# MinghanLi/STMask

Hardware: AMD Instinct MI355X
Metric: frames/sec at 360x640 R50-DCN-FPN (STMask hot path, fp32) (higher is better)
Workload: dtype f32

## Files before the change

include/stmask_hip.h:

```cpp
#ifndef STMASK_HIP_H_
#define STMASK_HIP_H_

#include <stddef.h>
#include <stdint.h>

#ifdef __cplusplus
extern "C" {
#endif

#define STM_ABI_VERSION 6

enum stm_status {
    STM_OK = 0,
    STM_EINVAL = -1,
    STM_ENULL = -2,
    STM_ELAUNCH = -3,
    STM_EWORKSPACE = -4,
    STM_EUNSUPPORTED = -5
};

typedef void* stm_stream_t;

int stm_version(void);
const char* stm_last_error_string(void);
// ... 150 lines not shown
int stm_conv_kxr_tile_pixels(int kw, int fmt, int channel_tiles);
size_t stm_conv_kxr_packed_bytes(const struct stm_conv_geom* g);
int stm_conv_pack_weights_kxr_f32(const float* weight, void* packed, const struct stm_conv_geom* g, float wscale, stm_stream_t stream);
int stm_conv2d_planar_kxr_f32(const void* x_planes, const void* packed_weight, const float* bias, float* out_f32, void* out_planes,
                              const struct stm_conv_geom* g, int relu, stm_stream_t stream);

size_t stm_chain_tail_weight_bytes(void);
size_t stm_chain_tail_weight_bytes_proj(void);
int stm_chain_pack_tail_f32(const float* w3, const float* w1_next, void* packed, float wscale3, float wscale1, stm_stream_t stream);
int stm_chain_pack_tail_proj_f32(const float* w3, const float* wds, const float* w1_next, void* packed, float wscale3, float wscale1,
                                 stm_stream_t stream);
int stm_bottleneck_chain_f32(const void* mid1_planes, const void* x_planes, void* y_planes, void* z_planes, const void* w2_packed,
                             const void* tail_packed, const float* b2, const float* b3, const float* b1_next, float out_scale2,
                             float out_scale3, float out_scale1, int B, int H, int W, stm_stream_t stream);
int stm_bottleneck_chain_proj_f32(const void* mid1_planes, const void* x0_planes, void* y_planes, void* z_planes, const void* w2_packed,
                                  const void* tail_packed, const float* b2, const float* b3, const float* b1_next, float out_scale2,
                                  float out_scale3, float out_scale1, int B, int H, int W, stm_stream_t stream);

size_t stm_conv_packed_weight_bytes(int Cout, int Cin, int kh, int kw, int planes);
int stm_conv_pack_weights_f32(const float* weight, void* packed, int Cout, int Cin, int kh, int kw, int planes,
                              stm_stream_t stream);
size_t stm_conv_packed_weight_bytes_tiled(int Cout, int Cin, int kh, int kw, int planes, int tile_n);
int stm_conv_pack_weights_tiled_f32(const float* weight, void* packed, int Cout, int Cin, int kh, int kw, int planes,
                                    int tile_n, stm_stream_t stream);
int stm_conv_pack_weights_fmt_f32(const float* weight, void* packed, int Cout, int Cin, int kh, int kw, int tile_n, int fmt,
                                  float wscale, stm_stream_t stream);
int stm_split_planes_fmt_f32(const float* x, void* planes, int64_t n_pixels, int C, int fmt, stm_stream_t stream);

int stm_split_bf16_planes_f32(const float* x , void* planes ,
                              int64_t n_pixels, int C, stm_stream_t stream);
int stm_conv2d_planar_f32(const void* x_planes, const void* packed_weight, const float* bias, const float* residual_f32,
                          const void* residual_planes, float* out_f32, void* out_planes, const stm_conv_geom* g, int relu,
                          stm_stream_t stream);
int stm_conv2d_planar_ws_f32(const void* x_planes, const void* packed_weight, const float* bias, const float* residual_f32,
                             const void* residual_planes, float* out_f32, void* out_planes, const stm_conv_geom* g, int relu,
                             void* workspace, size_t workspace_bytes, stm_stream_t stream);

int stm_gather_detections_f32(const int64_t* idx, const int64_t* cls, const float* score, const float* box, const int* count,
                              const float* mask_coeff, const float* track, const float* centerness, int B, int top_k, int N,
                              int mask_dim, int embed_dim, int D, float* out_box, int64_t* out_cls, float* out_score,
                              float* out_coeff, float* out_track, float* out_centerness, int* out_clip, stm_stream_t stream);
int stm_shift_rois_f32(const float* box, const int* clip, float* rois, int n, int feat_h, int feat_w, stm_stream_t stream);
int stm_shift_apply_f32(const float* loc_shift, const float* coeff_shift, float* box, float* coeff, float* score, int n,
                        int mask_dim, float score_decay, stm_stream_t stream);
int stm_match_scores_f32(const float* cos, const float* mask_iou, const float* det_box, const float* prev_box,
                         const float* det_score, const int64_t* det_cls, const int64_t* prev_cls, const int* det_clip,
                         const int* prev_offsets, int D, int Pn, const float* coeff4, float dummy_iou, int* match,
                         stm_stream_t stream);
int stm_match_scores_embed_f32(const float* det_track, const float* prev_track, int embed_dim, const float* mask_iou,
                               const float* det_box, const float* prev_box, const float* det_score, const int64_t* det_cls,
                               const int64_t* prev_cls, const int* det_clip, const int* prev_offsets, int D, int Pn,
                               const float* coeff4, float dummy_iou, int* match, stm_stream_t stream);
int stm_gather_rows2(const void* const* a_rows, const void* const* b_rows, void* const* out_rows, const int* row_bytes,
                     int n_tensors, const int* plan, int n_rows, int n_a, stm_stream_t stream);
int stm_pack_tracked_f32(const float* mask, const float* score, const int* tracked, const int* offsets, const float* box,
                         const int64_t* cls, const float* mask_coeff, int n_rows, int hw, int B, int top_k, int cols,
                         int mask_dim, int max_age, float score_thr, int* keep_ws, float* out, stm_stream_t stream);
int stm_pack_tracked_bits_f32(const uint64_t* mask_bits, int words, const float* score, const int* tracked, const int* offsets,
                              const float* box, const int64_t* cls, const float* mask_coeff, int n_rows, int B, int top_k,
                              int cols, int mask_dim, int max_age, float score_thr, int* keep_ws, float* out,
                              stm_stream_t stream);

int stm_split_planes_f16(const float* x, void* planes, int64_t n_pixels, int C, stm_stream_t stream);
int stm_conv_pack_weights_f16(const float* weight, void* packed, int Cout, int Cin, int kh, int kw, int tile_n, float wscale,
                              stm_stream_t stream);
int stm_conv2d_planar_f16(const void* x_planes, const void* packed_weight, const float* bias, const float* residual_f32,
// ... 169 lines not shown
```

stmask_amd/csrc/conv_bf16x.hip:

```cpp
#include "planar_common.h"
#include "conv_plan.h"
#include <stdarg.h>
#include <algorithm>
#include <array>
#include <type_traits>
#include <utility>
#include <atomic>

namespace {

static int* g_range_flags[STM_MAX_DEVICES] = {};
static int* current_range_flag()
{
    const int dev = stm_current_device();
    return dev >= 0 ? g_range_flags[dev] : nullptr;
}

struct PlanarArgs {
    const uint8_t* xp;
    const uint8_t* wp;
    const float* bias;
    const float* res_f32;
    const uint8_t* res_pl;
    float* out_f32;
// ... 190 lines not shown
    f16x8 r0[LPR], r1[LPR];
    if (pre) {
#pragma unroll
        for (int pass = 0; pass < LPR; ++pass) {
            const int m = min(m0 + wm * 64 + pass * (64 / LPR) + prow, a.M - 1);
            const size_t ri = (((size_t)(co >> 5) * a.res_np + m) * 32 + (co & 31)) * 2;
            r0[pass] = *reinterpret_cast<const f16x8*>(a.res_pl + ri);
            r1[pass] = fmt == 1 ? *reinterpret_cast<const f16x8*>(a.res_pl + ri + a.res_pstride) : r0[pass];
        }
    }
#pragma unroll
    for (int pass = 0; pass < LPR; ++pass) {
        const int pr = pass * (64 / LPR) + prow;
        const int m = m0 + wm * 64 + pr;
        if (m >= a.M) continue;
        const f32x4 v0 = *reinterpret_cast<const f32x4*>(park + pr * EP_LD + seg * 8);
        const f32x4 v1 = *reinterpret_cast<const f32x4*>(park + pr * EP_LD + seg * 8 + 4);
        float v[8] = {v0.x, v0.y, v0.z, v0.w, v1.x, v1.y, v1.z, v1.w};
#pragma unroll
        for (int e = 0; e < 8; ++e) v[e] = __builtin_fmaf(v[e], a.out_scale, bias8[e]);
        if (pre) epilogue_store8<false, FMT>(a, m, co, nvalid, v, true, r0[pass], r1[pass]);
        else epilogue_store8<false, FMT>(a, m, co, nvalid, v);
    }
}

__global__ __launch_bounds__(256) void planar_splitk_finish_kernel(const PlanarArgs a, int bn)
{
    const int segs_g = (a.cout_g + 7) >> 3;
    const int64_t idx = (int64_t)blockIdx.x * 256 + threadIdx.x;
    const int64_t total = (int64_t)a.M * a.groups * segs_g;
    if (idx >= total) return;
    const int sg = (int)(idx % (a.groups * segs_g));
    const int m = (int)(idx / (a.groups * segs_g));
    const int grp = sg / segs_g, cog = (sg - grp * segs_g) * 8;
    const int col = grp * a.ntpg * bn + cog;
    float v[8] = {0, 0, 0, 0, 0, 0, 0, 0};
    const float* p = a.partial + (size_t)m * a.ldp + col;
    const size_t pstride = (size_t)a.M * a.ldp;
    for (int k0 = 0; k0 < a.splitk; k0 += 4) {
        f32x4 q0[4], q1[4];
#pragma unroll
        for (int j = 0; j < 4; ++j) {
            const float* pk = p + (size_t)min(k0 + j, a.splitk - 1) * pstride;
            q0[j] = *reinterpret_cast<const f32x4*>(pk);
            q1[j] = *reinterpret_cast<const f32x4*>(pk + 4);
        }
#pragma unroll
        for (int j = 0; j < 4; ++j) {
            if (k0 + j < a.splitk) {
                v[0] += q0[j].x; v[1] += q0[j].y; v[2] += q0[j].z; v[3] += q0[j].w;
                v[4] += q1[j].x; v[5] += q1[j].y; v[6] += q1[j].z; v[7] += q1[j].w;
            }
        }
    }
    epilogue_store8(a, m, grp * a.cout_g + cog, min(8, a.cout_g - cog), v);
}

constexpr int POOL_BIG_SHIFT = 16;
constexpr float POOL_BIG_PIECE = (float)(1 << POOL_BIG_SHIFT);
template <bool BIG>
__device__ __forceinline__ bool pooled_walk(const PlanarArgs& a, unsigned long long* pool, int pool_ld, const float* park, int lane, int mw, int col)
{
    constexpr int EP_LD = 32 * 2 + 4;
    const int hw = a.Ho * a.Wo;
    const int rows = min(64, a.M - mw);
    int b = mw / hw, r = mw - b * hw;
// ... 17 lines not shown
                while (!__hip_atomic_compare_exchange_weak(word, &old, old + add, __ATOMIC_RELAXED, __ATOMIC_RELAXED, __HIP_MEMORY_SCOPE_AGENT)) {}
                const unsigned long long now = old + add, margin = (unsigned long long)a.win_hw << (32 + POOL_BIG_SHIFT);
                if ((now < old || now >= 0ull - margin) && a.range_flag) *reinterpret_cast<volatile int*>(a.range_flag) = 1;
            }
            sum = 0.0f;
            if (r == hw) { r = 0; ++b; }
        }
    }
    return any_big;
}
__device__ __forceinline__ void pooled_epilogue(const PlanarArgs& a, unsigned long long* pool, int pool_ld, uint8_t* smem, int wave, int lane, int mw, int col)
{
    const float* park = park_base<2>(smem, wave);
    asm volatile("s_waitcnt lgkmcnt(0)" ::: "memory");
    if (pooled_walk<false>(a, pool, pool_ld, park, lane, mw, col)) pooled_walk<true>(a, pool, pool_ld, park, lane, mw, col);
}

template <int NPL, int MG, int NJ, int DT = 0, int ST = 2, int ABL = 0, bool DUAL = false, int CLS = 0>
__global__ __launch_bounds__(512, 1) void conv_planar_kernel(const typename planar_args<CLS>::type a_in)
{
#if defined(__HIP_DEVICE_COMPILE__)
    extern __shared__ __align__(16) uint8_t smem[];
    constexpr int BM = CV_BM * MG;
    constexpr int BN = 64 * NJ;
    constexpr int WPL = BN * 64;
    constexpr int XBUF = NPL * BM * 64, WBUF = NPL * WPL, BUF = XBUF + WBUF;
    constexpr int NWAVES = 4 * MG;
    constexpr int WDMA = (BN / 16) * NPL / NWAVES;
    static_assert((BN / 16) * NPL % NWAVES == 0, "weight tile must split evenly over the waves");
    static_assert(ST == 2 || (ST == 3 && DT == 1 && NPL <= 2), "the three-buffer ring is built for the fp16 formats");

    int tiles_ = a_in.m_tiles * a_in.n_tiles * a_in.splitk;
    if constexpr (CLS) tiles_ = a_in.cls_tiles;
    else if (a_in.m_gate) tiles_ = min(a_in.m_tiles, (*a_in.m_gate + BM - 1) / BM) * a_in.n_tiles;
    const int tiles = tiles_;
    const int per_xcd = (tiles + 7) >> 3;
    if (!CLS && a_in.m_gate && (int)(blockIdx.x >> 3) >= per_xcd) return;
    int logical = (blockIdx.x & 7) * per_xcd + (blockIdx.x >> 3);
    if constexpr (CLS) {
        const int j = blockIdx.x >> 3;
        const int jm = j / a_in.n_tiles, nt_ = j - jm * a_in.n_tiles;
        logical = (jm * 8 + (int)(blockIdx.x & 7)) * a_in.n_tiles + nt_;
    }
    if (logical >= tiles) return;
    PlanarArgs a_cls;
    const PlanarArgs* ap = &a_in;
    if constexpr (CLS) {
        int c = 0;
#pragma unroll
        for (int i = 1; i < 9; ++i)
            if (i < a_in.n_cls && logical >= a_in.cls[i].tile0) c = i;
        a_cls = static_cast<const PlanarArgs&>(a_in);
        a_cls.wp = a_in.cls[c].wp;
        a_cls.kh = a_in.cls[c].kh; a_cls.kw = a_in.cls[c].kw; a_cls.ph = a_in.cls[c].ph; a_cls.pw = a_in.cls[c].pw;
        a_cls.Ho = a_in.cls[c].Ho; a_cls.Wo = a_in.cls[c].Wo; a_cls.M = a_in.cls[c].M;
        a_cls.slabs = a_in.cls[c].slabs; a_cls.kslabs = a_in.cls[c].slabs; a_cls.win_off = a_in.cls[c].win_off;
        a_cls.inv_hw = a_in.cls[c].inv_hw; a_cls.inv_w = a_in.cls[c].inv_w;
        if constexpr (CLS == 2) {
            a_cls.xp = a_in.xp + a_in.x_off[c];
            a_cls.plane_bytes = a_in.plane_bytes - (unsigned)a_in.x_off[c];
            a_cls.m_gate = a_in.gate[c];
        }
        logical -= a_in.cls[c].tile0;
        ap = &a_cls;
    }
    const PlanarArgs& a = *ap;
    const int ksp = a.splitk == 1 ? 0 : logical % a.splitk;
// ... 906 lines not shown
    }
    const int out_ld = g->out_ld ? g->out_ld : g->Cout, res_ld = g->res_ld ? g->res_ld : g->Cout;
    STM_REQUIRE(out_ld >= g->Cout && res_ld >= g->Cout, STM_EINVAL, "%s: bad leading dimensions out_ld=%d res_ld=%d", who, out_ld, res_ld);
    const bool win = g->n_levels <= 0 && g->win_w > 0;
    const int64_t out_rows = win ? (int64_t)g->B * g->win_h * g->win_w : M;
    const int64_t x_np = g->x_np ? g->x_np : in_pixels, out_np = g->out_np ? g->out_np : out_rows, res_np = g->res_np ? g->res_np : M;
    STM_REQUIRE(!win || (!c.residual_f32 && !c.residual_planes && !dual), STM_EUNSUPPORTED, "%s: window launches take no residual / second source", who);
    STM_REQUIRE(x_np >= in_pixels && out_np >= out_rows && res_np >= M, STM_EINVAL, "%s: x_np / out_np / res_np smaller than the pixel count", who);
    STM_REQUIRE((uintptr_t)c.x_planes % 16 == 0 && (uintptr_t)c.packed_weight % 16 == 0, STM_EINVAL,
                "%s: x_planes and packed_weight must be 16-byte aligned", who);
    if (dual) {
        STM_REQUIRE(groups == 1 && g->n_levels <= 0 && g->kh == 1 && g->kw == 1 && g->sh == 1 && g->sw == 1 && g->ph == 0 && g->pw == 0 &&
                    g->H == g->Ho && g->W == g->Wo && (g->fmt == 1 || g->fmt == 2), STM_EUNSUPPORTED,
                    "%s: 1x1 / stride 1 / one group / fp16 plane formats only", who);
        STM_REQUIRE(dual->C2 > 0 && dual->C2 % CV_BK == 0 && dual->C2 < g->C && dual->s2 >= 1 && dual->H2 > 0 && dual->W2 > 0 &&
                    (dual->H2 - 1) / dual->s2 + 1 == g->Ho && (dual->W2 - 1) / dual->s2 + 1 == g->Wo, STM_EINVAL,
                    "%s: second source %d channels of %dx%d at stride %d does not match the %dx%d output", who, dual->C2, dual->H2, dual->W2, dual->s2,
                    g->Ho, g->Wo);
    }
    const int64_t x_slabs = dual ? (int64_t)(g->C - dual->C2) / CV_BK : (int64_t)groups * (g->C / CV_BK);
    const int64_t plane_bytes = x_slabs * x_np * 64;
    STM_REQUIRE(plane_bytes < ((int64_t)1 << 31), STM_EUNSUPPORTED, "%s: plane larger than 2 GiB", who);
    STM_REQUIRE(M < ((int64_t)1 << 30), STM_EUNSUPPORTED, "%s: too many output pixels", who);
    const int64_t o_slabs = stm_cdiv(g->Cout, 32);
    const int64_t xps = g->x_plane_stride ? g->x_plane_stride : x_slabs * x_np * 32;
    const int64_t ops = g->out_plane_stride ? g->out_plane_stride : o_slabs * out_np * 32;
    const int64_t rps = g->res_plane_stride ? g->res_plane_stride : o_slabs * res_np * 32;
    STM_REQUIRE(xps % 8 == 0, STM_EINVAL, "%s: x_plane_stride must be a multiple of 8 elements", who);
    a.xp = static_cast<const uint8_t*>(c.x_planes); a.wp = static_cast<const uint8_t*>(c.packed_weight); a.bias = c.bias;
    a.res_f32 = c.residual_f32; a.res_pl = static_cast<const uint8_t*>(c.residual_planes);
    a.out_f32 = c.out_f32; a.out_pl = static_cast<uint8_t*>(c.out_planes);
    a.B = g->B; a.H = g->H; a.W = g->W; a.C = g->C; a.Ho = g->Ho; a.Wo = g->Wo; a.Cout = g->Cout;
    a.kh = g->kh; a.kw = g->kw; a.sh = g->sh; a.sw = g->sw; a.ph = g->ph; a.pw = g->pw;
    a.out_ld = out_ld; a.res_ld = res_ld; a.relu = c.relu;
    a.x_np = (int)x_np; a.out_np = (int)out_np; a.res_np = (int)res_np;
    a.M = (int)M; a.n_tiles = stm_cdiv(g->Cout, bn); a.m_tiles = 0; a.slabs = g->kh * g->kw * (g->C / CV_BK);
    a.plane_bytes = (unsigned)plane_bytes;
    a.x_pstride = xps * 2; a.out_pstride = ops * 2; a.res_pstride = rps * 2;
    a.groups = groups; a.cout_g = cout_g; a.ntpg = stm_cdiv(cout_g, bn);
    for (int i = 0; i < 8; ++i) a.group_real[i] = (i < groups && g->group_cout[i] > 0 && g->group_cout[i] < cout_g) ? g->group_cout[i] : cout_g;
    a.n_levels = g->n_levels > 0 ? g->n_levels : 0;
    for (int l = 0; l < 8; ++l) { a.lvl_start[l] = g->lvl_start[l]; a.lvl_h[l] = g->lvl_h[l]; a.lvl_w[l] = g->lvl_w[l]; }
    a.lvl_start[8] = g->lvl_start[8];
    a.vec_epilogue = (cout_g % 8 == 0) && (!c.out_f32 || out_ld % 4 == 0) && (!c.residual_f32 || res_ld % 4 == 0) && ((uintptr_t)c.out_f32 % 16 == 0) &&
                     ((uintptr_t)c.out_planes % 16 == 0) && ((uintptr_t)c.residual_f32 % 16 == 0) && ((uintptr_t)c.residual_planes % 16 == 0) &&
                     (ops % 8 == 0) && (rps % 8 == 0);
    STM_REQUIRE(g->kh * g->kw <= 32, STM_EUNSUPPORTED, "%s: more than 32 taps", who);
    a.pointwise = (g->n_levels <= 0 && !win && g->kh == 1 && g->kw == 1 && g->sh == 1 && g->sw == 1 && g->ph == 0 && g->pw == 0) ? 1 : 0;
    a.win_w = win ? g->win_w : 0; a.win_hw = win ? g->win_h * g->win_w : 0; a.win_off = win ? g->win_y0 * g->win_w + g->win_x0 : 0;
    a.inv_hw = g->n_levels > 0 ? 0.0f : 1.0f / (float)((int64_t)g->Ho * g->Wo);
    a.inv_w = g->n_levels > 0 ? 0.0f : 1.0f / (float)g->Wo;
    STM_REQUIRE(g->n_levels > 0 || M < ((int64_t)1 << 24), STM_EUNSUPPORTED, "%s: more than 2^24 output pixels in one launch", who);
    a.fmt = (g->fmt >= 0 && g->fmt <= 2) ? g->fmt : 0;
    a.out_fmt = g->out_fmt_plus1 > 0 ? g->out_fmt_plus1 - 1 : a.fmt;
    STM_REQUIRE(a.out_fmt >= 0 && a.out_fmt <= 2 && (a.out_fmt == a.fmt || (a.fmt == 2 && a.out_fmt == 1)), STM_EINVAL,
                "%s: output format %d cannot be produced by a format-%d layer", who, a.out_fmt, a.fmt);
    a.out_scale = (a.fmt >= 1 && g->out_scale > 0.0f) ? g->out_scale : 1.0f;
    a.range_flag = current_range_flag();
    const int want_planes = a.fmt == 0 ? 3 : (a.fmt == 1 ? 2 : 1);
    STM_REQUIRE(g->planes == want_planes || (a.fmt == 0 && g->planes == 2), STM_EINVAL, "%s: format %d has %d planes (planes = %d)", who, a.fmt,
                want_planes, g->planes);
    a.splitk = 1; a.kslabs = a.slabs; a.partial = nullptr; a.ldp = a.n_tiles * bn;
    a.m_gate = gate;
    STM_REQUIRE(!gate || !wset || !wset->pool, STM_EUNSUPPORTED, "%s: pooled window sets take no pixel gate", who);
    a.xp2 = nullptr; a.x2_pstride = 0; a.plane2_bytes = 0; a.c1_slabs = a.slabs; a.x2_np = 0; a.H2 = a.W2 = 0; a.s2 = 1;
    if (dual) {
        const int64_t in2 = (int64_t)g->B * dual->H2 * dual->W2;
        const int64_t np2 = dual->x2_np ? dual->x2_np : in2;
        const int64_t slabs2 = dual->C2 / CV_BK;
        const int64_t ps2 = dual->x2_plane_stride ? dual->x2_plane_stride : slabs2 * np2 * 32;
        STM_REQUIRE(np2 >= in2 && slabs2 * np2 * 64 < ((int64_t)1 << 31) && ps2 % 8 == 0 && (uintptr_t)dual->x2 % 16 == 0, STM_EINVAL,
                    "%s: bad second-source plane geometry", who);
        a.xp2 = static_cast<const uint8_t*>(dual->x2); a.x2_pstride = ps2 * 2; a.plane2_bytes = (unsigned)(slabs2 * np2 * 64);
        a.c1_slabs = (int)x_slabs; a.x2_np = (int)np2; a.H2 = dual->H2; a.W2 = dual->W2; a.s2 = dual->s2;
    }
    bool full = cout_g % 64 == 0;
    for (int gi = 0; gi < groups && gi < 8; ++gi) full = full && a.group_real[gi] == cout_g;
    f = ConvFacts{bn, a.fmt, g->planes, groups, cout_g, full, a.slabs, a.kh, a.kw, a.sh, a.sw, a.ph, a.pw, M, a.n_tiles, dual != nullptr, win, gate != nullptr,
                  c.workspace && (uintptr_t)c.workspace % 16 == 0, c.workspace_bytes, a.ldp};
    return STM_OK;
}

bool window_inside(const stm_conv_window& w, const stm_conv_geom* g)
{
    return w.Ho > 0 && w.Wo > 0 && w.y0 >= 0 && w.x0 >= 0 && w.y0 + w.Ho <= g->win_h && w.x0 + w.Wo <= g->win_w;
}
bool window_taps_inside(const stm_conv_window& w, const stm_conv_geom* g) { return conv_plan::taps_inside(w.kh, w.kw, w.ph, w.pw, w.Ho, w.Wo, g->H, g->W); }

int64_t fill_cls(PlanarArgsCls::Cls& c, const void* packed, const stm_conv_window& w, const stm_conv_geom* g, int images, int row0, int tile0)
{
    const int64_t Mc = (int64_t)images * w.Ho * w.Wo;
    c.wp = static_cast<const uint8_t*>(packed);
    c.kh = w.kh; c.kw = w.kw; c.ph = w.ph; c.pw = w.pw; c.Ho = w.Ho; c.Wo = w.Wo; c.M = (int)Mc;
    c.slabs = w.kh * w.kw * (g->C / CV_BK);
    c.win_off = row0 + w.y0 * g->win_w + w.x0;
    c.inv_hw = 1.0f / (float)(w.Ho * w.Wo); c.inv_w = 1.0f / (float)w.Wo;
    c.tile0 = tile0;
    return Mc;
}

int build_gated_set(const ConvCall& c, const char* who, const ConvFacts& f, const int* gate, Launch& l)
{
    const stm_conv_geom* const g = c.g;
    const WinSet* const wset = c.wset;
    PlanarArgsSeg& as = l.args;
    STM_REQUIRE(f.bn == 128 && as.fmt == 1 && !c.dual && f.win, STM_EUNSUPPORTED, "%s: window sets run on the 256 x 128 ring tiles of the fp16x2 format", who);
    STM_REQUIRE(g->B % wset->n == 0, STM_EINVAL, "%s: %d images are not %d equal segments", who, g->B, wset->n);
    const int seg_b = g->B / wset->n;
    as.m_gate = nullptr;
    as.pool = nullptr; as.pool_ld = 0;
    int t0 = 0;
    for (int i = 0; i < 9; ++i) {
// ... 34 lines not shown
        STM_REQUIRE((int64_t)g->B * w.Ho * w.Wo < ((int64_t)1 << 24), STM_EUNSUPPORTED, "%s: more than 2^24 output pixels in one window", who);
        const int k = conv_plan::window_takes_kx3(tn, w.kh, w.kw, w.ph, w.pw, w.Ho, w.Wo, g->H, g->W) ? 1 : 0;
        const int64_t Mc = fill_cls(L[k].args.cls[ncls[k]++], wset->packed[i], w, g, g->B, 0, t0[k]);
        t0[k] += stm_cdiv(Mc, 2 * CV_BM) * f.n_tiles;
    }
    for (int k = 0; k < 2; ++k) {
        if (!ncls[k]) continue;
        PlanarArgsCls& ac = L[k].args;
        for (int i = ncls[k]; i < 9; ++i) ac.cls[i] = ac.cls[0];
        ac.pool = wset->pool;
        ac.pool_ld = g->Cout;
        ac.n_cls = ncls[k];
        ac.cls_tiles = t0[k];
        L[k].plan = conv_plan::plan_window_set(k == 1, 1, k == 0 ? CLS_ABL : 0, t0[k], f.n_tiles, ac.kslabs);
        L[k].planned = true;
    }
    return STM_OK;
}

int conv2d_planar_impl(const ConvCall& c, stm_stream_t stream)
{
    const char* who = c.dual ? "stm_conv2d_planar_dual_f32" : "stm_conv2d_planar_f32";
    const int* const gate = stm_internal_take_pixel_gate();
    Launch L[2];
    PlanarArgs& a = L[0].args;
    ConvFacts f;
    int rc = planar_validate(c, who, gate, a, f);
    if (rc != STM_OK) return rc;
    if (c.wset) {
        rc = gate ? build_gated_set(c, who, f, gate, L[0]) : build_window_set(c, who, f, tunables(), L);
        if (rc != STM_OK) return rc;
    } else {
        const ConvPlan& p = L[0].plan = conv_plan::plan_conv(f, tunables());
        a.m_tiles = p.m_tiles; a.splitk = p.splitk; a.kslabs = p.kslabs;
        if (p.splitk > 1) a.partial = static_cast<float*>(c.workspace);
        L[0].planned = true;
    }
    for (const Launch& l : L) {
        if (!l.planned) continue;
        rc = run_launch(l, stream);
        if (rc != STM_OK) return rc;
    }
    if (a.splitk < 2) return STM_OK;
    const int64_t total = (int64_t)a.M * a.groups * ((a.cout_g + 7) / 8);
    if (t_plan_text) { t_plan_text->add("planar_splitk_finish_kernel grid=%d block=256 lds=0\n", stm_cdiv(total, 256)); return STM_OK; }
    hipLaunchKernelGGL(planar_splitk_finish_kernel, dim3(stm_cdiv(total, 256)), dim3(256), 0, stm_hs(stream), a, f.bn);
    STM_CHECK_LAUNCH("planar_splitk_finish_kernel");
    return STM_OK;
}

stm_conv_geom window0_geom(const stm_conv_geom* g, const stm_conv_window& w)
{
    stm_conv_geom g0 = *g;
    g0.kh = w.kh; g0.kw = w.kw; g0.ph = w.ph; g0.pw = w.pw;
    g0.Ho = w.Ho; g0.Wo = w.Wo; g0.win_y0 = w.y0; g0.win_x0 = w.x0;
    return g0;
}
}

extern "C" int stm_conv2d_planar_ws_f32(const void* x_planes, const void* packed_weight, const float* bias, const float* residual_f32,
                                        const void* residual_planes, float* out_f32, void* out_planes, const stm_conv_geom* g,
                                        int relu, void* workspace, size_t workspace_bytes, stm_stream_t stream)
{
    return conv2d_planar_impl({x_planes, packed_weight, bias, residual_f32, residual_planes, out_f32, out_planes, g, relu, workspace, workspace_bytes,
                               nullptr, nullptr}, stream);
}
// ... 93 lines not shown
```

stmask_amd/csrc/conv_plan.h:

```cpp
#pragma once
#include <algorithm>
#include <cstddef>
#include <cstdint>

namespace conv_plan {

constexpr int CV_RING64_SMALL = 512;
constexpr int CV_SK_TARGET = 256;
struct ConvTunables {
    int ring = 3;
    int ring64 = 3;
    int splitk = 0;
    int mg = 0;
    int abl = 0;
    int kx3 = 1;
};

constexpr int BM = 128;
constexpr int KX3_WBUF = 2 * 128 * 64;
constexpr int KX3_LDS_LOOP = 2 * 2 * 272 * 64 + 3 * KX3_WBUF;

inline int cdiv(int64_t a, int64_t b) { return (int)((a + b - 1) / b); }

struct ConvFacts {
    int bn;
    int fmt, planes;
    int groups, cout_g;
    bool full;
    int slabs;
    int kh, kw, sh, sw, ph, pw;
    int64_t M;
    int n_tiles;
    bool dual, win, gated;
    bool ws_usable;
    size_t ws_bytes;
    int ldp;
};

struct ConvPlan {
    bool kx3 = false;
    int npl = 0, mg = 0, nj = 0, dt = 0, st = 0, abl = 0;
    bool dual = false;
    int cls = 0;
    int m_tiles = 0, splitk = 1, kslabs = 0;
    unsigned grid = 0, block = 0;
    size_t lds = 0;
};

inline size_t planar_lds(int npl, int mg, int nj, int st)
{
    size_t lds = (size_t)st * (npl * BM * mg * 64 + npl * (64 * nj) * 64);
    const size_t park = (size_t)4 * mg * 64 * (32 * nj + 4) * sizeof(float);
    return lds < park ? park : lds;
}
inline size_t kx3_lds(bool win)
{
    if (win) return 2 * 2 * 384 * 64 + 3 * KX3_WBUF;
    return std::max<size_t>(8 * 64 * (64 + 4) * sizeof(float), (size_t)KX3_LDS_LOOP);
}

inline void plan_splitk(ConvPlan& p, const ConvFacts& f, const ConvTunables& tn, int tiles)
{
    if (f.gated) return;
    int sk = tn.splitk;
    if (sk <= 0) {
        sk = 1;
        if (f.bn == 64) {
            if (!f.full) {
                if (tiles <= 256 && f.slabs >= 24) sk = (int)std::min<int64_t>(std::min<int64_t>(8, 768 / tiles), f.slabs / 10);
            } else if (tiles <= 128 && f.slabs >= 24)
                sk = (int)std::min<int64_t>(std::min<int64_t>(8, CV_SK_TARGET / tiles), f.slabs / (tiles <= 40 ? 10 : 16));
        } else if (tiles < 128 && f.slabs >= 24) sk = (int)std::min<int64_t>(std::min<int64_t>(8, 256 / tiles), f.slabs / 12);
    }
    if (sk < 2) return;
    const int per = cdiv(f.slabs, sk);
    sk = cdiv(f.slabs, per);
    if (sk < 2 || !f.ws_usable || (size_t)sk * f.M * f.ldp * sizeof(float) > f.ws_bytes) return;
    p.splitk = sk; p.kslabs = per;
}

inline ConvPlan plan_conv(const ConvFacts& f, const ConvTunables& tn)
{
    ConvPlan p;
    p.npl = f.fmt == 2 ? 1 : (f.fmt == 1 ? 2 : (f.planes == 3 ? 3 : 2));
    p.dt = f.fmt >= 1 ? 1 : 0;
    p.dual = f.dual;
    p.kslabs = f.slabs;
    if (f.bn == 64) {
        p.mg = 1; p.nj = 1;
        p.m_tiles = cdiv(f.M, BM);
        plan_splitk(p, f, tn, p.m_tiles * f.n_tiles);
        const int tiles = p.m_tiles * f.n_tiles * p.splitk;
        const bool small_grid = tiles <= CV_RING64_SMALL;
        const bool ring = f.full && (tn.ring64 == 3 ? (small_grid || (p.splitk == 1 && f.slabs >= 12 && f.slabs <= 40)) : tn.ring64 == 4);
        p.st = (f.fmt >= 1 && ring) ? 3 : 2;
        p.grid = 8 * cdiv(tiles, 8);
    } else {
        const int64_t t2 = (int64_t)cdiv(f.M, 2 * BM) * f.n_tiles;
        p.mg = tn.mg ? tn.mg : (t2 >= 192 ? 2 : 1);
        p.nj = 2;
        p.m_tiles = cdiv(f.M, BM * p.mg);
        plan_splitk(p, f, tn, p.m_tiles * f.n_tiles);
        const int tiles = p.m_tiles * f.n_tiles * p.splitk;
        const bool ring = tn.ring == 3;
        p.grid = 8 * cdiv(tiles, 8);
#ifdef STM_ABLATE
        if (f.fmt == 1 && ring && p.mg == 2 && tn.abl) {
            const int abl = tn.abl;
            p.abl = (abl == 1 || abl == 2 || abl == 3 || abl == 5 || abl == 8 || abl == 16 || abl == 32 || abl == 64) ? abl : 7;
            p.st = 3; p.dual = false;
// ... 39 lines not shown
```

stmask_amd/planar.py:

```python
import ctypes
import functools
import os
from typing import Any, NamedTuple, Optional

import torch
import torch.nn.functional as F

from . import _lib, ops
from ._lib import StmError, call
from .ops import _pair


FMT = 0
BACKBONE_FMT = None

TILE64_MAX_SLABS = 8
FCB_PLANAR = True
STEM_PLANAR = True
C3DS_FUSED = True
STEM_FUSED = True
CONV_KXR = True
TN_BORDER = True
TN_POOL = True
CONV_CHAIN = True
# ... 148 lines not shown
        if out_planes is not None:
            g.out_np, g.out_plane_stride = out_planes.shape[2], out_planes.shape[1] * out_planes.shape[2] * 32
            if out_slab_off < 0 or out_slab_off + -(-self.O // 32) > out_planes.shape[1]:
                raise StmError(f"PlanarConv: {self.O} output channels from slab {out_slab_off} run past the {out_planes.shape[1]} slabs of out_planes")
            p_pl = out_planes.data_ptr() + (out_slab_off * g.out_np + out_off_p) * 64
        if out_f32 is not None:
            g.out_ld = out_f32.shape[-1]
            p_f32 = out_f32.data_ptr() + (out_off_f * g.out_ld + out_ch_off) * 4
        r32 = rpl = 0
        if residual is not None:
            if residual.dtype == dt:
                if residual.shape[0] < NP:
                    raise StmError(f"PlanarConv: residual has {residual.shape[0]} plane(s), format {self.fmt} reads {NP}")
                g.res_np, g.res_plane_stride = residual.shape[2], residual.shape[1] * residual.shape[2] * 32
                rpl = residual.data_ptr()
            else:
                g.res_ld = residual.shape[-1]
                r32 = residual.data_ptr()
        started = _timing_start()
        x_ptr = xp.data_ptr() + ((x_ch_off // 32) * N + x_off) * 64
        if use_kxr:
            g.fmt = self.fmt
            if "kxr" not in self._packed:
                ops.planar_range_flag()
                self._packed["kxr"] = ops.conv_pack_weights_kxr(self.weight, g, wscale=self.wscale)
            packed, g.out_scale = self._packed["kxr"]
            if gate is not None:
                ops.conv_set_pixel_gate(*gate)
            call("stm_conv2d_planar_kxr_f32", x_ptr, ops._p(packed), ops._p(self.bias), p_f32, p_pl, ctypes.byref(g), 1 if self.relu else 0, ops._stream())
        else:
            packed = self.packed(g.tile_n)
            g.fmt, g.out_scale = self.fmt, self.out_scale
            g.out_fmt_plus1 = 0 if self.out_fmt == self.fmt else self.out_fmt + 1
            ws = ops._workspace(self.SPLITK_WS_BYTES, dev, "conv_splitk") if splitk and gate is None else None
            if gate is not None:
                if x2 is not None:
                    raise StmError("PlanarConv: gated launches take no second source")
                ops.conv_set_pixel_gate(*gate)
            if x2 is not None:
                p2, H2, W2, s2 = x2
                if p2.dtype != dt or p2.dim() != 4 or p2.shape[0] < NP or p2.shape[3] != 32 or not p2.is_contiguous() or shape[0] != "img":
                    raise StmError("PlanarConv: the second source must be contiguous planes of this layer's format over one image size")
                call("stm_conv2d_planar_dual_f32", x_ptr, ops._p(p2), p2.shape[1] * 32, H2, W2, s2, p2.shape[2], p2.shape[1] * p2.shape[2] * 32,
                     ops._p(packed), ops._p(self.bias), r32, rpl, p_f32, p_pl, ctypes.byref(g), 1 if self.relu else 0, ops._p(ws), ws.numel(), ops._stream())
            else:
                call("stm_conv2d_planar_ws_f32", x_ptr, ops._p(packed), ops._p(self.bias), r32, rpl, p_f32, p_pl, ctypes.byref(g), 1 if self.relu else 0,
                     ops._p(ws), ws.numel() if ws is not None else 0, ops._stream())
        if started is not None:
            _timing_stop(started, 2.0 * M * self.O * self.C * self.kh * self.kw * self.algo_frac, (M, self.C, self.O, self.kh, self.sh, self.groups, g.tile_n),
                         {0: 6 if self.planes == 3 else 3, 1: 3, 2: 1}[self.fmt], self.role, self._algo_bytes(M, shape, NP, NPo, dt, out_f32, out_planes, residual))
        if out == "both":
            return out_f32, out_planes
        return out_f32 if out == "f32" else out_planes

    def window_segments(self, xp, B, H, W, windows, out_planes, out_hw, gate, x_ch_off=0, out_slab_off=0):
        if self.fmt != 1 or self.out_fmt != 1 or (self.sh, self.sw) != (1, 1):
            raise StmError("PlanarConv.window_segments: fp16x2 planes and stride 1 only")
        S, N = xp.shape[1], xp.shape[2]
        n = len(windows)
        if xp.dim() != 4 or not xp.is_contiguous() or B % n or B * H * W > N or x_ch_off % 32 or S * 32 < x_ch_off + self.groups * self.C:
            raise StmError(f"PlanarConv.window_segments: {B} images of {H}x{W} in {n} segments do not fit planes {tuple(xp.shape)}")
        if (out_planes.shape[2] < B * out_hw * out_hw or out_slab_off < 0 or out_slab_off + self.O // 32 > out_planes.shape[1] or self.O % 128
                or (H - self.kh + 1, W - self.kw + 1) != (out_hw, out_hw)):
            raise StmError("PlanarConv.window_segments: the output planes do not hold the layer's valid convolution")
        packed = self.packed(128)
        g = _lib.ConvGeom()
        g.B, g.H, g.W, g.C, g.Cout, g.sh, g.sw, g.planes, g.fmt, g.tile_n = B, H, W, self.C, self.O, 1, 1, 2, 1, 128
        g.groups, g.win_h, g.win_w, g.out_scale = self.groups, out_hw, out_hw, self.out_scale
        g.x_np, g.x_plane_stride = N, S * N * 32
        g.out_np, g.out_plane_stride = out_planes.shape[2], out_planes.shape[1] * out_planes.shape[2] * 32
        wins = (_lib.ConvWindow * n)()
        for i, (ho, wo, y0, x0) in enumerate(windows):
            wins[i].kh, wins[i].kw, wins[i].ph, wins[i].pw, wins[i].Ho, wins[i].Wo, wins[i].y0, wins[i].x0 = self.kh, self.kw, -y0, -x0, ho, wo, y0, x0
        g.kh, g.kw, g.Ho, g.Wo = self.kh, self.kw, windows[0][0], windows[0][1]
        ptrs = (ctypes.c_void_p * n)(*[packed.data_ptr()] * n)
        started = _timing_start()
        ops.conv_set_pixel_gate(*gate)
        call("stm_conv2d_planar_windows_f32", xp.data_ptr() + (x_ch_off // 32) * N * 64, ptrs, wins, n, ops._p(self.bias), None,
             out_planes.data_ptr() + out_slab_off * g.out_np * 64, ctypes.byref(g), 1 if self.relu else 0, ops._stream())
# ... 11 lines not shown
    def _algo_bytes(self, M, shape, NP, NPo, dt, out_f32, out_planes, residual):
        in_px = M if shape[0] == "levels" else shape[1] * shape[2] * shape[3]
        nbytes = in_px * self.groups * self.C * 2 * NP + self.weight.numel() * 2 * NP
        if out_planes is not None:
            nbytes += M * self.O * 2 * NPo
        if out_f32 is not None:
            nbytes += M * self.O * 4
        if residual is not None:
            nbytes += M * self.O * (2 * NP if residual.dtype == dt else 4)
        return nbytes


def _nhwc(t):
    return t.permute(0, 2, 3, 1).contiguous()


def _split(t_nhwc, fmt=None):
    return ops.split_planes(t_nhwc, FMT if fmt is None else fmt)


@functools.lru_cache(maxsize=None)
def head_split_default():
    return os.environ.get("STM_HEAD_SPLIT", "1") != "0"


@functools.lru_cache(maxsize=None)
def head_shapes_default():
    return os.environ.get("STM_HEAD_SHAPES", "1") != "0"


@functools.lru_cache(maxsize=None)
def head_center_default():
    return os.environ.get("STM_HEAD_CENTER", "1") != "0"


class HeadOutputs(NamedTuple):
    small: PlanarConv
    trk: PlanarConv
    fa: Optional[Any] = None
    fconv: Optional[PlanarConv] = None
    adconv: Optional[PlanarConv] = None
    adfused: Optional[PlanarConv] = None


class _Levels(NamedTuple):
    B: int
    sizes: tuple
    starts: tuple
    ntot: int
    dev: torch.device

    @property
    def lv(self):
        return ("levels", self.B, self.sizes)


class PlanarGraph:
    GROUP_PAD = 64

    def __init__(self, net):
        cfg = net.cfg
        self.net = net
        self.fmt = FMT
        fpn = net.fpn
        self.n_lat = len(fpn.lat_layers)
        self.fpn_pred = [PlanarConv(m.weight, m.bias, m.stride, m.padding, relu=True) for m in fpn.pred_layers]
# ... 54 lines not shown
                           group_cout=[sum(m.weight.shape[0] for m in grp) for grp in mods])
        tr = head.track_layer[k]
        trk = PlanarConv(tr.weight, tr.bias, 1, tr.padding, relu=False)
        if not self.fcb:
            return HeadOutputs(small, trk)
        fa = head.conf_layer[k]
        n_c = fa.conv.weight.shape[0]
        n_cp = -(-n_c // 16) * 16
        assert n_cp <= P
        fconv = PlanarConv(F.pad(fa.conv.weight, (0, 0, 0, 0, 0, 0, 0, n_cp - n_c)), F.pad(fa.conv.bias, (0, n_cp - n_c)), 1, fa.conv.padding,
                           relu=False, tile_n=64, group_cout=[n_c], algo_frac=n_c / n_cp)
        ad = fa.conv_adaption
        O, Cin, akh, akw = ad.weight.shape
        adconv = adfused = None
        if ad.deform_groups == 1 and Cin == 256 and akh * akw in (9, 15):
            wk = ad.weight.detach().permute(0, 2, 3, 1).reshape(O, akh * akw * Cin, 1, 1)
            adconv = PlanarConv(wk, None, 1, 0, relu=True)
            if DCN_FUSED and FCB_FUSED and self.fmt in (1, 2) and ops.deform_conv_fused_supported(Cin, O, (akh, akw), False, self.fmt):
                adfused = PlanarConv(ad.weight, None, 1, fa.padding, relu=True)
        return HeadOutputs(small, trk, fa, fconv, adconv, adfused)

    SPARSE_SIDES = (9, 7, 5)

    def sparse_supported(self):
        return self.head_planar and not self.fcb and self.head.num_priors == 1

    def sparse_capacity(self, B, sizes):
        s0, s1, s2 = self.SPARSE_SIDES
        per_frame = max(1, 2 * sum(h * w for h, w in sizes) // (s1 * s1 + s2 * s2))
        return -(-per_frame * B // 256) * 256

    @staticmethod
    def sparse_segment_capacity(cap):
        return min(cap, -(-cap // (2 * 256)) * 256)

    def _build_sparse(self):
        if self._sparse_layers is not None:
            return self._sparse_layers
        P = self.GROUP_PAD
        cw = self.tower2.O // 4

        def cut(layer, rows, **kw):
            c = PlanarConv(layer.weight[rows], layer.bias[rows], 1, (layer.ph, layer.pw), relu=layer.relu, fmt=layer.fmt, **kw)
            c.wscale = ops._pow2_wscale(layer.weight) if layer.fmt >= 1 else None
            return c

        t1c, t1r = cut(self.tower1, slice(0, cw)), cut(self.tower1, slice(cw, 4 * cw))
        t2c, t2r = cut(self.tower2, slice(0, cw)), cut(self.tower2, slice(cw, 4 * cw), groups=3)
        cls, small = [], []
        for sm in (f.small for f in self.finals):
            gc = sm.group_cout
            cls.append(cut(sm, slice(0, P), tile_n=64, group_cout=gc[:1], algo_frac=gc[0] / float(P)))
            small.append(cut(sm, slice(P, 3 * P), groups=2, tile_n=64, group_cout=gc[1:], algo_frac=sum(gc[1:]) / (2.0 * P)))
        self._sparse_layers = (t1c, t1r, t2c, t2r, cls, small)
        self._split_layers = (cut(self.tower1, slice(cw, 2 * cw)), cut(self.tower1, slice(2 * cw, 4 * cw)),
                              cut(self.tower2, slice(cw, 2 * cw)), cut(self.tower2, slice(2 * cw, 4 * cw), groups=2))
        return self._sparse_layers

    def _sparse_head(self, up, g, toc):
        head, (B, sizes, _, ntot, dev) = self.head, g
        thresh, cap = self.sparse[:2]
        center = self.sparse[2] if len(self.sparse) > 2 else head_center_default()
        split = len(self.sparse) > 3 and bool(self.sparse[3])
        own = ops.HEAD_CTL_OWN if split else 0
        if cap is None:
            cap = self.sparse_capacity(B, sizes)
        if len(self.sparse) > 4 and bool(self.sparse[4]) and split and center and self.fmt == 1:
# ... 64 lines not shown
        cw, P = self.tower2.O // 4, self.GROUP_PAD
        S0, S1, S2 = self.SPARSE_SIDES
        NP, pdt = ops.plane_layout(self.fmt)
        kx = ntot >= self.finals[0].small.kxr_rule_pixels()
        x = t1c(up, lv, out="planes", splitk=False)
        x = t2c(x, lv, out="planes", splitk=False)
        cls = [c(x, lv, out="f32", splitk=False, kxr=kx) for c in cls_l]
        toc("head_towers")
        shp = [(c.kh, c.kw) for c in small_l]
        if any(c.kh > S2 or c.kw > S2 or not (c.kh & c.kw & 1) or (t.kh, t.kw) != (c.kh, c.kw) for c, t in zip(small_l, trk_l)):
            raise StmError("sparse head: an output layer's kernel does not fit the patch maps")
        w1 = [(kh + 2, kw + 2, (S2 - kh) // 2, (S2 - kw) // 2) for kh, kw in shp]
        w2 = [(kh, kw, (S2 - kh) // 2, (S2 - kw) // 2) for kh, kw in shp]
        lst, ctl = ops.head_candidates(cls, head.num_classes, thresh, cap, [h * w for h, w, _, _ in w1], [h * w for h, w, _, _ in w2], B, sizes,
                                       split=True, shapes=True)
        tot = K * cap
        patch = ops.head_patch_gather(up, torch.empty(NP, cw // 32, tot * S0 * S0, 32, device=dev, dtype=pdt), S0, cap, B, sizes, lst, ctl, segs=K)
        x1 = torch.empty(NP, 3 * cw // 32, tot * S1 * S1, 32, device=dev, dtype=pdt)
        xq = torch.empty(NP, 3 * cw // 32, tot * S2 * S2, 32, device=dev, dtype=pdt)
        seg, own = ops.HEAD_CTL_SEG, ops.HEAD_CTL_OWN
        t1b.window_segments(patch, tot, S0, S0, w1, x1, S1, (ctl, seg + ops.HEAD_CTL_GATE_A))
        t1m.window_segments(patch, tot, S0, S0, w1, x1, S1, (ctl, seg + own + ops.HEAD_CTL_GATE_A), out_slab_off=cw // 32)
        ops.head_patch_mask(x1, S1, cap, B, sizes, lst, ctl, segs=K)
        t2b.window_segments(x1, tot, S1, S1, w2, xq, S2, (ctl, seg + ops.HEAD_CTL_GATE_B))
        t2m.window_segments(x1, tot, S1, S1, w2, xq, S2, (ctl, seg + own + ops.HEAD_CTL_GATE_B), x_ch_off=cw, out_slab_off=cw // 32)
        ops.head_patch_mask(xq, S2, cap, B, sizes, lst, ctl, segs=K)
        c2 = S2 // 2

        def centre(c, k, blk, **kw):
            return c(xq, ("img", cap, S2, S2), x_off=k * cap * S2 * S2, out="f32", out_f32=torch.empty(cap, c.O, device=dev),
                     window=(0, 0, 1, 1, c.ph - c2, c.pw - c2, 1, 1), gate=(ctl, seg * (k + 1) + blk + ops.HEAD_CTL_GATE_POS), **kw)

        small = [centre(c, k, 0, kxr=kx) for k, c in enumerate(small_l)]
        trk = [centre(c, k, own, x_ch_off=2 * cw, kxr=False) for k, c in enumerate(trk_l)]
        gd = (ctl, ops.HEAD_CTL_DENSE)
        x = t1r(up, lv, out="planes", gate=gd)
        x = t2r(x, lv, out="planes", gate=gd)
        small_d = [c(x, lv, out="f32", gate=gd, kxr=kx) for c in small_l]
        trk_d = [c(x, lv, out="f32", x_ch_off=2 * cw, gate=gd) for c in trk_l]
        toc("head_finals")
        out = ops.head_assemble_sparse(cls, small, trk, small_d, trk_d, B, sizes, head.num_classes, head.mask_dim, head.embed_dim, P,
                                       1, 0, lst, ctl, cap, split=True, shapes=True)
        self.sparse_ctl, self.sparse_list, self.sparse_segments = ctl[:ops.HEAD_CTL_SEG], None, (ctl, lst, cap)
        return out

    @property
    def sparse_list(self):
        if self._sparse_list is not None or self.sparse_segments is None:
            return self._sparse_list
        ctl, lst, cap = self.sparse_segments
        c, seg, own = ctl.tolist(), ops.HEAD_CTL_SEG, ops.HEAD_CTL_OWN
        K = len(c) // seg - 1
        n = [(c[seg * (k + 1) + own + ops.HEAD_CTL_N], c[seg * (k + 1) + ops.HEAD_CTL_N]) for k in range(K)]
        return torch.cat([lst[k * cap:k * cap + no] for k, (no, _) in enumerate(n)] + [lst[k * cap + no:k * cap + na] for k, (no, na) in enumerate(n)])

    @sparse_list.setter
    def sparse_list(self, lst):
        self._sparse_list = lst
        if lst is not None:
            self.sparse_segments = None

    def run(self, bb_outs, planes=None):
        toc = self.timer.toc if self.timer is not None else (lambda name: None)
        toc("backbone")
        lat, latp, B, sizes = self._fpn_laterals(bb_outs, planes)
        toc("fpn_lateral")
        for d in self.fpn_down:
# ... 586 lines not shown
```

Measured before the change: 1869.

## Allow split-K on gated conv launches and enlarge sparse segment capacity

Result: no change. 1869 (-0.0%).

```diff
diff --git a/include/stmask_hip.h b/include/stmask_hip.h
--- a/include/stmask_hip.h
+++ b/include/stmask_hip.h
@@ -206,6 +206,8 @@
 int stm_conv2d_planar_f32(const void* x_planes, const void* packed_weight, const float* bias, const float* residual_f32,
                           const void* residual_planes, float* out_f32, void* out_planes, const stm_conv_geom* g, int relu,
                           stm_stream_t stream);
+#define STM_CONV_RELU 1
+#define STM_CONV_GATED_SPLITK 2
 int stm_conv2d_planar_ws_f32(const void* x_planes, const void* packed_weight, const float* bias, const float* residual_f32,
                              const void* residual_planes, float* out_f32, void* out_planes, const stm_conv_geom* g, int relu,
                              void* workspace, size_t workspace_bytes, stm_stream_t stream);
diff --git a/stmask_amd/csrc/conv_bf16x.hip b/stmask_amd/csrc/conv_bf16x.hip
--- a/stmask_amd/csrc/conv_bf16x.hip
+++ b/stmask_amd/csrc/conv_bf16x.hip
@@ -246,6 +246,7 @@
     if (idx >= total) return;
     const int sg = (int)(idx % (a.groups * segs_g));
     const int m = (int)(idx / (a.groups * segs_g));
+    if (a.m_gate && m >= *a.m_gate) return;
     const int grp = sg / segs_g, cog = (sg - grp * segs_g) * 8;
     const int col = grp * a.ntpg * bn + cog;
     float v[8] = {0, 0, 0, 0, 0, 0, 0, 0};
@@ -329,7 +330,7 @@
 
     int tiles_ = a_in.m_tiles * a_in.n_tiles * a_in.splitk;
     if constexpr (CLS) tiles_ = a_in.cls_tiles;
-    else if (a_in.m_gate) tiles_ = min(a_in.m_tiles, (*a_in.m_gate + BM - 1) / BM) * a_in.n_tiles;
+    else if (a_in.m_gate) tiles_ = min(a_in.m_tiles, (*a_in.m_gate + BM - 1) / BM) * a_in.n_tiles * a_in.splitk;
     const int tiles = tiles_;
     const int per_xcd = (tiles + 7) >> 3;
     if (!CLS && a_in.m_gate && (int)(blockIdx.x >> 3) >= per_xcd) return;
@@ -1302,7 +1303,7 @@
     a.out_f32 = c.out_f32; a.out_pl = static_cast<uint8_t*>(c.out_planes);
     a.B = g->B; a.H = g->H; a.W = g->W; a.C = g->C; a.Ho = g->Ho; a.Wo = g->Wo; a.Cout = g->Cout;
     a.kh = g->kh; a.kw = g->kw; a.sh = g->sh; a.sw = g->sw; a.ph = g->ph; a.pw = g->pw;
-    a.out_ld = out_ld; a.res_ld = res_ld; a.relu = c.relu;
+    a.out_ld = out_ld; a.res_ld = res_ld; a.relu = c.relu & STM_CONV_RELU;
     a.x_np = (int)x_np; a.out_np = (int)out_np; a.res_np = (int)res_np;
     a.M = (int)M; a.n_tiles = stm_cdiv(g->Cout, bn); a.m_tiles = 0; a.slabs = g->kh * g->kw * (g->C / CV_BK);
     a.plane_bytes = (unsigned)plane_bytes;
@@ -1347,7 +1348,7 @@
     bool full = cout_g % 64 == 0;
     for (int gi = 0; gi < groups && gi < 8; ++gi) full = full && a.group_real[gi] == cout_g;
     f = ConvFacts{bn, a.fmt, g->planes, groups, cout_g, full, a.slabs, a.kh, a.kw, a.sh, a.sw, a.ph, a.pw, M, a.n_tiles, dual != nullptr, win, gate != nullptr,
-                  c.workspace && (uintptr_t)c.workspace % 16 == 0, c.workspace_bytes, a.ldp};
+                  c.workspace && (uintptr_t)c.workspace % 16 == 0, c.workspace_bytes, a.ldp, gate && (c.relu & STM_CONV_GATED_SPLITK)};
     return STM_OK;
 }
 
@@ -1448,6 +1449,7 @@
         if (rc != STM_OK) return rc;
     } else {
         const ConvPlan& p = L[0].plan = conv_plan::plan_conv(f, tunables());
+        STM_REQUIRE(!p.refused, STM_EINVAL, "%s: %s", who, p.refused);
         a.m_tiles = p.m_tiles; a.splitk = p.splitk; a.kslabs = p.kslabs;
         if (p.splitk > 1) a.partial = static_cast<float*>(c.workspace);
         L[0].planned = true;
diff --git a/stmask_amd/csrc/conv_plan.h b/stmask_amd/csrc/conv_plan.h
--- a/stmask_amd/csrc/conv_plan.h
+++ b/stmask_amd/csrc/conv_plan.h
@@ -35,6 +35,7 @@
     bool ws_usable;
     size_t ws_bytes;
     int ldp;
+    bool gate_split = false;
 };
 
 struct ConvPlan {
@@ -45,6 +46,7 @@
     int m_tiles = 0, splitk = 1, kslabs = 0;
     unsigned grid = 0, block = 0;
     size_t lds = 0;
+    const char* refused = nullptr;
 };
 
 inline size_t planar_lds(int npl, int mg, int nj, int st)
@@ -59,23 +61,30 @@
     return std::max<size_t>(8 * 64 * (64 + 4) * sizeof(float), (size_t)KX3_LDS_LOOP);
 }
 
+inline int splitk_rule(const ConvFacts& f, int tiles)
+{
+    int sk = 1;
+    if (f.bn == 64) {
+        if (!f.full) {
+            if (tiles <= 256 && f.slabs >= 24) sk = (int)std::min<int64_t>(std::min<int64_t>(8, 768 / tiles), f.slabs / 10);
+        } else if (tiles <= 128 && f.slabs >= 24)
+            sk = (int)std::min<int64_t>(std::min<int64_t>(8, CV_SK_TARGET / tiles), f.slabs / (tiles <= 40 ? 10 : 16));
+    } else if (tiles < 128 && f.slabs >= 24) sk = (int)std::min<int64_t>(std::min<int64_t>(8, 256 / tiles), f.slabs / 12);
+    return sk;
+}
 inline void plan_splitk(ConvPlan& p, const ConvFacts& f, const ConvTunables& tn, int tiles)
 {
-    if (f.gated) return;
-    int sk = tn.splitk;
-    if (sk <= 0) {
-        sk = 1;
-        if (f.bn == 64) {
-            if (!f.full) {
-                if (tiles <= 256 && f.slabs >= 24) sk = (int)std::min<int64_t>(std::min<int64_t>(8, 768 / tiles), f.slabs / 10);
-            } else if (tiles <= 128 && f.slabs >= 24)
-                sk = (int)std::min<int64_t>(std::min<int64_t>(8, CV_SK_TARGET / tiles), f.slabs / (tiles <= 40 ? 10 : 16));
-        } else if (tiles < 128 && f.slabs >= 24) sk = (int)std::min<int64_t>(std::min<int64_t>(8, 256 / tiles), f.slabs / 12);
-    }
+    if (f.gated && !f.gate_split) return;
+    int sk = tn.splitk > 0 ? tn.splitk : splitk_rule(f, tiles);
     if (sk < 2) return;
+    if (f.gated && tn.splitk > 0 && (sk > f.slabs || f.slabs % sk)) { p.refused = "the forced K parts do not divide the K-slabs of a gated split launch"; return; }
     const int per = cdiv(f.slabs, sk);
     sk = cdiv(f.slabs, per);
-    if (sk < 2 || !f.ws_usable || (size_t)sk * f.M * f.ldp * sizeof(float) > f.ws_bytes) return;
+    if (sk < 2) return;
+    if (!f.ws_usable || (size_t)sk * f.M * f.ldp * sizeof(float) > f.ws_bytes) {
+        if (f.gated) p.refused = "a gated split-K launch needs a 16-byte aligned workspace of parts x capacity pixels x padded channels floats";
+        return;
+    }
     p.splitk = sk; p.kslabs = per;
 }
 
diff --git a/stmask_amd/planar.py b/stmask_amd/planar.py
--- a/stmask_amd/planar.py
+++ b/stmask_amd/planar.py
@@ -204,7 +204,9 @@
             packed = self.packed(g.tile_n)
             g.fmt, g.out_scale = self.fmt, self.out_scale
             g.out_fmt_plus1 = 0 if self.out_fmt == self.fmt else self.out_fmt + 1
-            ws = ops._workspace(self.SPLITK_WS_BYTES, dev, "conv_splitk") if splitk and gate is None else None
+            gated_split = gate is not None and splitk == "gate"
+            ws = ops._workspace(self.SPLITK_WS_BYTES, dev, "conv_splitk") if splitk and (gate is None or gated_split) else None
+            relu_bits = (1 if self.relu else 0) | (2 if gated_split else 0)
             if gate is not None:
                 if x2 is not None:
                     raise StmError("PlanarConv: gated launches take no second source")
@@ -216,7 +218,7 @@
                 call("stm_conv2d_planar_dual_f32", x_ptr, ops._p(p2), p2.shape[1] * 32, H2, W2, s2, p2.shape[2], p2.shape[1] * p2.shape[2] * 32,
                      ops._p(packed), ops._p(self.bias), r32, rpl, p_f32, p_pl, ctypes.byref(g), 1 if self.relu else 0, ops._p(ws), ws.numel(), ops._stream())
             else:
-                call("stm_conv2d_planar_ws_f32", x_ptr, ops._p(packed), ops._p(self.bias), r32, rpl, p_f32, p_pl, ctypes.byref(g), 1 if self.relu else 0,
+                call("stm_conv2d_planar_ws_f32", x_ptr, ops._p(packed), ops._p(self.bias), r32, rpl, p_f32, p_pl, ctypes.byref(g), relu_bits,
                      ops._p(ws), ws.numel() if ws is not None else 0, ops._stream())
         if started is not None:
             _timing_stop(started, 2.0 * M * self.O * self.C * self.kh * self.kw * self.algo_frac, (M, self.C, self.O, self.kh, self.sh, self.groups, g.tile_n),
@@ -294,6 +296,11 @@
 @functools.lru_cache(maxsize=None)
 def head_center_default():
     return os.environ.get("STM_HEAD_CENTER", "1") != "0"
+
+
+@functools.lru_cache(maxsize=None)
+def head_gated_splitk_default():
+    return os.environ.get("STM_HEAD_GATED_SPLITK", "0") == "1"
 
 
 class HeadOutputs(NamedTuple):
@@ -414,7 +421,7 @@
 
     @staticmethod
     def sparse_segment_capacity(cap):
-        return min(cap, -(-cap // (2 * 256)) * 256)
+        return min(cap, -(-2 * cap // (3 * 256)) * 256)
 
     def _build_sparse(self):
         if self._sparse_layers is not None:
@@ -545,7 +552,8 @@
                      window=(0, 0, 1, 1, c.ph - c2, c.pw - c2, 1, 1), gate=(ctl, seg * (k + 1) + blk + ops.HEAD_CTL_GATE_POS), **kw)
 
         small = [centre(c, k, 0, kxr=kx) for k, c in enumerate(small_l)]
-        trk = [centre(c, k, own, x_ch_off=2 * cw, kxr=False) for k, c in enumerate(trk_l)]
+        trk_sk = "gate" if head_gated_splitk_default() else True
+        trk = [centre(c, k, own, x_ch_off=2 * cw, kxr=False, splitk=trk_sk) for k, c in enumerate(trk_l)]
         gd = (ctl, ops.HEAD_CTL_DENSE)
         x = t1r(up, lv, out="planes", gate=gd)
         x = t2r(x, lv, out="planes", gate=gd)
```
